# tsolomko/SWCompression

Hardware: NVIDIA H100
Metric: decompressed_GB_per_s (higher is better)
Workload: dtype u8

## Files before the change

swcompression_b200/csrc/inflate.cu:

```cuda
#include <cstdlib>
#include <cstring>
#include "common.cuh"
#include "inflate.cuh"
#include "host_util.h"

namespace swc {
namespace inflate {

namespace k2 {
constexpr int WARPS = 8;
constexpr int CTAS_PER_SM = 4;
constexpr u32 RING = 2048;
constexpr u32 SPAN = RING / 2;
constexpr u32 LITBUF = SPAN + 32;
struct __align__(16) WarpSmem {
    uint4 stage[32];
    u8 ring[RING];
    u8 lit[LITBUF];
};
}

__global__ void __launch_bounds__(k2::WARPS * 32, k2::CTAS_PER_SM)
lz_resolve_kernel(BatchArgs a) {
    using namespace k2;
    __shared__ WarpSmem smem[WARPS];
    const u64 unit = ((u64)blockIdx.x * blockDim.x + threadIdx.x) >> 5;
    if (unit >= a.n) return;
    if (a.status[unit] != SWC_OK) return;
    const u32 nrec = a.rec_count[unit];
    if (nrec == REC_DIRECT) return;
    WarpSmem &S = smem[(threadIdx.x >> 5) & (WARPS - 1)];
    const u32 lane = threadIdx.x & 31;
    const u32 sub = lane >> 2, t = lane & 3;
    const u64 off = a.out_off[unit];
    const u32 len = (u32)a.out_len[unit];
    u8 *out = a.out_base + off;
    const u32 *rec = a.rec_base + rec_start(off + a.out_cap[unit]);
    const u8 *lits = (const u8 *)(a.rec_base + rec_start(off));
    const u32 ph = (u32)((uintptr_t)out & 15);
    const u32 M = RING - 1;
    u32 done = 0;
    u32 flushed = 0;
    u32 lit = 0;
    u32 g = 0;
    u32 part = 0;
    auto flush = [&](u32 to) {
        const u32 c0 = (flushed + ph) >> 4, c1 = (to + ph + 15) >> 4;
        for (u32 c = c0 + lane; c < c1; c += 32) {
            const int cs = (int)(c * 16) - (int)ph;
            const u32 lo = cs < (int)flushed ? flushed : (u32)cs, hi = (u32)(cs + 16) < to ? (u32)(cs + 16) : to;
            if ((int)lo == cs && hi == (u32)(cs + 16)) {
                *(uint4 *)(out + cs) = *(const uint4 *)(S.ring + ((c * 16) & M));
            } else {
                for (u32 p = lo; p < hi; p++) out[p] = S.ring[(p + ph) & M];
            }
        }
        flushed = to;
    };
    for (;;) {
        const bool real = g + lane < nrec;
        u32 rv = REC_ESC;
        if (real) rv = *(rec - 1 - (g + lane));
        const Match m = get_match(rv);
        const u32 adv = m.adv - (lane == 0 ? part : 0u);
        const u32 run = adv - m.len;
        u32 end = adv, lend = run;
#pragma unroll
        for (int d = 1; d < 32; d <<= 1) {
            const u32 v = __shfl_up_sync(SWC_FULL, end, d), w = __shfl_up_sync(SWC_FULL, lend, d);
            if (lane >= (u32)d) { end += v; lend += w; }
        }
        const u32 k = __popc(__ballot_sync(SWC_FULL, real && end <= SPAN));
        u32 span, nl;
        u32 delta;
        if (k > 0) {
            span = __shfl_sync(SWC_FULL, end, k - 1);
            nl = __shfl_sync(SWC_FULL, lend, k - 1);
            delta = done + end - adv - (lend - run);
            if (lane >= k) lend = 0xFFFFFFFFu;
            g += k;
            part = 0;
        } else {
            const u32 adv0 = __shfl_sync(SWC_FULL, adv, 0);
            const u32 rem = g < nrec ? adv0 : len - done;
            if (rem == 0) break;
            span = nl = rem < SPAN ? rem : SPAN;
            if (g < nrec) part += span;
            delta = done;
            lend = lane == 0 ? nl : 0xFFFFFFFFu;
        }
        S.stage[lane] = make_uint4(done + end - m.len, lane < k ? m.len : 0u, m.dist, 0u);
        const uintptr_t lsrc = (uintptr_t)(lits + lit);
        const uint4 *lchunk = (const uint4 *)(lsrc & ~(uintptr_t)15);
        const u32 lofs = (u32)(lsrc & 15), nch = (lofs + nl + 15) >> 4;
        for (u32 c = lane; c < nch; c += 32) ((uint4 *)S.lit)[c] = __ldg(lchunk + c);
        __syncwarp();
        for (u32 j0 = 0; j0 < nl; j0 += 32) {
            const u32 j = j0 + lane;
            u32 r = 0;
#pragma unroll
            for (u32 step = 16; step > 0; step >>= 1)
                if (__shfl_sync(SWC_FULL, lend, r + step - 1) <= j) r += step;
            const u32 p = j + __shfl_sync(SWC_FULL, delta, r);
            if (j < nl) S.ring[(p + ph) & M] = S.lit[lofs + j];
        }
        lit += nl;
        const u32 bend = done + span;
        __syncwarp();
        auto src_byte = [&](u32 q) -> u8 { return q + RING >= bend ? S.ring[(q + ph) & M] : out[q]; };
#pragma unroll 1
        for (u32 b0 = 0; b0 < k; b0 += 8) {
            const uint4 rc = S.stage[b0 + sub];
            const u32 s = rc.x, l = rc.y, d = rc.z;
            const u32 src_end = s - d + (l < d ? l : d);
            bool pend = l != 0;
            u32 pmask = __ballot_sync(SWC_FULL, pend && t == 0);
            while (pmask) {
                const u32 oldest = (__ffs(pmask) - 1) >> 2;
                const u32 frontier = S.stage[b0 + oldest].x;
                const bool ready = pend && (sub == oldest || src_end <= frontier);
                if (ready) {
                    const u32 q0 = s - d;
                    if (d >= l) {
                        for (u32 i = t; i < l; i += 16) {
                            const bool p1 = i + 4 < l, p2 = i + 8 < l, p3 = i + 12 < l;
                            const u8 v0 = src_byte(q0 + i);
                            u8 v1 = 0, v2 = 0, v3 = 0;
                            if (p1) v1 = src_byte(q0 + i + 4);
                            if (p2) v2 = src_byte(q0 + i + 8);
                            if (p3) v3 = src_byte(q0 + i + 12);
                            S.ring[(s + i + ph) & M] = v0;
                            if (p1) S.ring[(s + i + 4 + ph) & M] = v1;
                            if (p2) S.ring[(s + i + 8 + ph) & M] = v2;
                            if (p3) S.ring[(s + i + 12 + ph) & M] = v3;
                        }
                    } else {
                        for (u32 i = t; i < l; i += 4) S.ring[(s + i + ph) & M] = src_byte(q0 + i % d);
                    }
                    pend = false;
                }
                __syncwarp();
                pmask = __ballot_sync(SWC_FULL, pend && t == 0);
            }
        }
        done = bend;
        __syncwarp();
        const u32 to = ((done + ph) & ~15u) - ph;
        if (done + ph >= 16 && to > flushed) flush(to);
        __syncwarp();
    }
    flush(len);
}

int launch(const BatchArgs &a, cudaStream_t stream) {
    if (a.n == 0) return SWC_OK;
    static const int forced = [] {
        const char *e = getenv("SWC_DEFLATE_K1");
        return !e ? -1 : !strcmp(e, "lut") ? 0 : !strcmp(e, "warp") ? 1 : -1;
    }();
    const bool use_lut = forced >= 0 ? forced == 0 : a.n >= 20000;
    SWC_CUDA_TRY(cudaMemsetAsync(a.ticket, 0, 16, stream));
    timing_mark(stream);
    const int st = use_lut ? launch_lut(a, stream) : launch_warp(a, stream);
    if (st) return st;
    timing_mark(stream);
    launch_slow(a, stream);
    timing_mark(stream);
    const u64 per_cta = k2::WARPS;
    lz_resolve_kernel<<<(unsigned)((a.n + per_cta - 1) / per_cta), k2::WARPS * 32, 0, stream>>>(a);
    count_launch();
    timing_mark(stream);
    SWC_CUDA_TRY(cudaGetLastError());
    return SWC_OK;
}

}
}
```

Measured before the change: 124.7.

## Stage far-match sources and literals into shared memory with cp.async

Before each batch, the source bytes of matches whose source lies outside the shared ring are bulk-copied into a per-warp shared buffer with cp.async. Literals are also loaded with cp.async, and the next round's records are prefetched a loop iteration early. The match copy loop then reads only shared memory, with each thread handling four contiguous bytes instead of four strided ones. This replaces scattered byte-wise global reads with 16-byte async copies. The cost is more shared memory per warp, plus an extra prefix scan and per-lane chunk-copy loop that can serialise when one lane has many chunks.

```diff
diff --git a/swcompression_b200/csrc/inflate.cu b/swcompression_b200/csrc/inflate.cu
--- a/swcompression_b200/csrc/inflate.cu
+++ b/swcompression_b200/csrc/inflate.cu
@@ -13,11 +13,18 @@
 constexpr u32 RING = 2048;
 constexpr u32 SPAN = RING / 2;
 constexpr u32 LITBUF = SPAN + 32;
+constexpr u32 FARBUF = 128 * 16;
+constexpr u32 NEAR = 0xFFFFFFFFu;
 struct __align__(16) WarpSmem {
     uint4 stage[32];
     u8 ring[RING];
     u8 lit[LITBUF];
+    u8 far[FARBUF];
 };
+__device__ __forceinline__ void cp_async16(void *dst, const void *src) {
+    asm volatile("cp.async.cg.shared.global [%0], [%1], 16;\n" ::"r"((u32)__cvta_generic_to_shared(dst)), "l"(src) : "memory");
+}
+__device__ __forceinline__ void cp_async_wait_all() { asm volatile("cp.async.wait_all;\n" ::: "memory"); }
 }
 
 __global__ void __launch_bounds__(k2::WARPS * 32, k2::CTAS_PER_SM)
@@ -57,10 +64,9 @@
         }
         flushed = to;
     };
+    u32 rv = lane < nrec ? __ldg(rec - 1 - lane) : REC_ESC;
     for (;;) {
         const bool real = g + lane < nrec;
-        u32 rv = REC_ESC;
-        if (real) rv = *(rec - 1 - (g + lane));
         const Match m = get_match(rv);
         const u32 adv = m.adv - (lane == 0 ? part : 0u);
         const u32 run = adv - m.len;
@@ -89,11 +95,34 @@
             delta = done;
             lend = lane == 0 ? nl : 0xFFFFFFFFu;
         }
-        S.stage[lane] = make_uint4(done + end - m.len, lane < k ? m.len : 0u, m.dist, 0u);
+        if (k > 0) rv = g + lane < nrec ? __ldg(rec - 1 - (g + lane)) : REC_ESC;
+        const u32 bend = done + span;
         const uintptr_t lsrc = (uintptr_t)(lits + lit);
-        const uint4 *lchunk = (const uint4 *)(lsrc & ~(uintptr_t)15);
+        const u8 *lchunk = (const u8 *)(lsrc & ~(uintptr_t)15);
         const u32 lofs = (u32)(lsrc & 15), nch = (lofs + nl + 15) >> 4;
-        for (u32 c = lane; c < nch; c += 32) ((uint4 *)S.lit)[c] = __ldg(lchunk + c);
+        for (u32 c = lane; c < nch; c += 32) cp_async16(S.lit + c * 16, lchunk + c * 16);
+        const u32 ms = done + end - m.len, mq = ms - m.dist;
+        const bool far = lane < k && m.len != 0 && mq + RING < bend;
+        const u32 c0 = (mq + ph) >> 4;
+        const u32 fch = far ? ((mq + m.len - 1 + ph) >> 4) - c0 + 1 : 0u;
+        u32 fend = fch;
+#pragma unroll
+        for (int d = 1; d < 32; d <<= 1) {
+            const u32 v = __shfl_up_sync(SWC_FULL, fend, d);
+            if (lane >= (u32)d) fend += v;
+        }
+        const u32 fbeg = fend - fch;
+        const u8 *outa = out - ph;
+        for (u32 c = 0; c < fch; c++) {
+            u8 *dst = S.far + (fbeg + c) * 16;
+            if (c0 + c > 0 || ph == 0) {
+                cp_async16(dst, outa + (c0 + c) * 16);
+            } else {
+                for (u32 b = ph; b < 16; b++) dst[b] = outa[b];
+            }
+        }
+        S.stage[lane] = make_uint4(ms, lane < k ? m.len : 0u, m.dist, far ? fbeg * 16 + ((mq + ph) & 15) : NEAR);
+        cp_async_wait_all();
         __syncwarp();
         for (u32 j0 = 0; j0 < nl; j0 += 32) {
             const u32 j = j0 + lane;
@@ -105,14 +134,17 @@
             if (j < nl) S.ring[(p + ph) & M] = S.lit[lofs + j];
         }
         lit += nl;
-        const u32 bend = done + span;
-        __syncwarp();
-        auto src_byte = [&](u32 q) -> u8 { return q + RING >= bend ? S.ring[(q + ph) & M] : out[q]; };
+        __syncwarp();
 #pragma unroll 1
         for (u32 b0 = 0; b0 < k; b0 += 8) {
             const uint4 rc = S.stage[b0 + sub];
             const u32 s = rc.x, l = rc.y, d = rc.z;
             const u32 src_end = s - d + (l < d ? l : d);
+            const bool fr = rc.w != NEAR;
+            const u8 *sb = fr ? S.far : S.ring;
+            const u32 s0 = fr ? rc.w : s - d + ph, sm = fr ? 0xFFFFFFFFu : M;
+            const u32 alim = fr ? FARBUF : M - 3;
+            auto src_byte = [&](u32 i) -> u8 { return sb[(s0 + i) & sm]; };
             bool pend = l != 0;
             u32 pmask = __ballot_sync(SWC_FULL, pend && t == 0);
             while (pmask) {
@@ -120,22 +152,35 @@
                 const u32 frontier = S.stage[b0 + oldest].x;
                 const bool ready = pend && (sub == oldest || src_end <= frontier);
                 if (ready) {
-                    const u32 q0 = s - d;
                     if (d >= l) {
-                        for (u32 i = t; i < l; i += 16) {
-                            const bool p1 = i + 4 < l, p2 = i + 8 < l, p3 = i + 12 < l;
-                            const u8 v0 = src_byte(q0 + i);
-                            u8 v1 = 0, v2 = 0, v3 = 0;
-                            if (p1) v1 = src_byte(q0 + i + 4);
-                            if (p2) v2 = src_byte(q0 + i + 8);
-                            if (p3) v3 = src_byte(q0 + i + 12);
-                            S.ring[(s + i + ph) & M] = v0;
-                            if (p1) S.ring[(s + i + 4 + ph) & M] = v1;
-                            if (p2) S.ring[(s + i + 8 + ph) & M] = v2;
-                            if (p3) S.ring[(s + i + 12 + ph) & M] = v3;
+                        for (u32 i = 4 * t; i < l; i += 16) {
+                            const bool p1 = i + 1 < l, p2 = i + 2 < l, p3 = i + 3 < l;
+                            const u32 a = (s0 + i) & sm, b = (s + i + ph) & M;
+                            u32 v0, v1 = 0, v2 = 0, v3 = 0;
+                            if (a <= alim && b <= M - 3) {
+                                const u8 *src = sb + a;
+                                u8 *dst = S.ring + b;
+                                v0 = src[0];
+                                if (p1) v1 = src[1];
+                                if (p2) v2 = src[2];
+                                if (p3) v3 = src[3];
+                                dst[0] = v0;
+                                if (p1) dst[1] = v1;
+                                if (p2) dst[2] = v2;
+                                if (p3) dst[3] = v3;
+                            } else {
+                                v0 = src_byte(i);
+                                if (p1) v1 = src_byte(i + 1);
+                                if (p2) v2 = src_byte(i + 2);
+                                if (p3) v3 = src_byte(i + 3);
+                                S.ring[b] = v0;
+                                if (p1) S.ring[(b + 1) & M] = v1;
+                                if (p2) S.ring[(b + 2) & M] = v2;
+                                if (p3) S.ring[(b + 3) & M] = v3;
+                            }
                         }
                     } else {
-                        for (u32 i = t; i < l; i += 4) S.ring[(s + i + ph) & M] = src_byte(q0 + i % d);
+                        for (u32 i = t; i < l; i += 4) S.ring[(s + i + ph) & M] = src_byte(i % d);
                     }
                     pend = false;
                 }
```

Measured after the change: 147.2, median of 6. 18.1% higher.
